# MasterVVK/qwen3-tts-axera-russian

Measured on AMD Instinct MI355X. Metric: 12Hz codec-tokens/s (codec frames/s, 16 codes each) + RTF, Qwen3-TTS-0.6B, higher is better.
Workload: dtype f16 weights/KV, f32 accumulate (talker+CP); vocoder exact fp32 (f32 MFMA); 1 GPU; configs[2]/[3]: batch=32 mixed ru/en prompts per GPU, 64 frames/utterance/step (prefill + hipGraph decode loop), utterance-sharded DP over 1 GPU(s); batch_per_gpu=32

## Files before the change

### qwen3_tts_axera_russian_amd/build.py

```python
from __future__ import annotations

import os
import shutil
import subprocess
import sys

HERE = os.path.dirname(os.path.abspath(__file__))
CSRC = os.path.join(HERE, "csrc")
LIB = os.path.join(HERE, "lib")
SOURCES = ["q3_common.cpp", "q3_formats.cpp", "q3_kernels.hip", "q3_model.hip", "q3_talker_api.hip", "q3_cp_api.hip",
           "q3_engine.hip", "q3_voc_kernels.hip", "q3_voc.hip", "q3_voc_stream.hip", "q3_enc.hip", "q3_enc_stream.hip",
           "q3_text_api.hip"]
TEST_SOURCES = ["q3_test_api.hip"]
ARCH = os.environ.get("Q3_OFFLOAD_ARCH", "gfx950")
EXTRA = os.environ.get("Q3_EXTRA_HIPCC_FLAGS", "-mllvm -amdgpu-kernarg-preload-count=16").split()


def _newer(dst: str, srcs) -> bool:
    if not os.path.exists(dst):
        return False
    t = os.path.getmtime(dst)
    return all(os.path.getmtime(s) <= t for s in srcs)


NO_SPILL = ("resunit_kernel", "linear_kernelILi1ELi1E", "linear_kernelILi1ELi2E", "linear_kernelILi2ELi1E",
            "linear_kernelILi2ELi2E", "attn_kernel", "attn_short_kernel", "cp_argmax_kernel", "talker_sample_kernel",
            "voc_attn_incr_kernel", "voc_incr_prepend_kernel", "voc_incr_emit_kernel", "voc_incr_prepend_split_kernel",
            "enc_conv_in_kernel", "enc_stream_unfold_kernel", "enc_stream_emit_kernel",
            "enc_stream_conv_in_kernel")


def kernel_resources(lib_path: str):
    import re
    import struct
    import tempfile
    readelf = "/opt/rocm/lib/llvm/bin/llvm-readelf"
    d = open(lib_path, "rb").read()
    res = {}
    i = d.find(b"__CLANG_OFFLOAD_BUNDLE__")
    while i >= 0:
        n = struct.unpack_from("<Q", d, i + 24)[0]
# ... 95 lines not shown
```

### qwen3_tts_axera_russian_amd/csrc/q3_cp_api.hip

```cpp
#include "../../include/qwen3tts_cp.h"
#include "q3_cp.h"

namespace q3 {

static bool two_row_enabled() {
    static const bool on = !(getenv("Q3_CP_TWO_ROW") && atoi(getenv("Q3_CP_TWO_ROW")) == 0);
    return on;
}

int cp_seed_row0(const Work& w, int R, int row0, int R_total) {
    (void)R;
    (void)row0;
    if (R_total <= 0) R_total = R;
    const int B16 = (R_total + 15) / 16 * 16;
    const bool two = two_row_enabled() && 2 * B16 <= w.max_rows;
    return two ? B16 : 0;
}

int cp_frame(hipStream_t s, const Model& m, Work& w, KVCache& kv, int R, const CpFrameIO& io, int row0, int R_total) {
    const ModelCfg& c = m.cfg;
    if (R_total <= 0) R_total = R;
    const int H = c.hidden, G = c.cp_groups;
    const int seed0 = cp_seed_row0(w, R, row0, R_total);
    RowMap rm;
// ... 36 lines not shown
        r2.pos = w.map_pos;
        r2.same_slot_rows = true;
        r2.valid_mod = R16;
        r2.valid_n = R;
        if (run_stack(s, m, m.cp, w, kv, R16 + R, r2, 256, 0)) return -1;
    } else {
        rm.pos_base = 0;
        if (run_stack(s, m, m.cp, w, kv, R, rm, 256, row0)) return -1;
        if (launch_gather_embed(s, m.talker_emb, c.talker_vocab, H, io.codes, 0, io.n_frames, io.frame_cap, 0, w.h, w.ssq, R,
                                row0, R_total, io.forced, w.xh, m.cp.L[0].in_ln))
            return -1;
        rm.pos_base = 1;
        if (run_stack(s, m, m.cp, w, kv, R, rm, 256, row0)) return -1;
    }
    const bool qkv_tab = m.cp_qkv_serves(R);
    for (int g = 0; g < G; g++) {
        if (g > 0) {
            rm.pos_base = g + 1;
            rm.skip_qkv0 = qkv_tab;
            if (run_stack(s, m, m.cp, w, kv, R, rm, 256, row0)) return -1;
        }
        LinArgs a;
        a.wp = m.cp_head[g].wp;
        a.N = c.cp_vocab;
        a.K = H;
        a.M = row0 + R;
        a.m_begin = row0;
        a.nt = 0;
        a.x16 = w.xh;
        a.ssq = w.ssq;
        a.ssq_parts = H / 16;
        a.eps = c.eps;
        a.y = w.logits;
        a.ldy = c.cp_vocab;
// ... 13 lines not shown
        x.top_k = io.top_k;
        x.seed = io.seed;
        x.seed_ptr = io.seed_ptr;
        x.forced = io.forced;
        x.slots = io.slots;
        if (g + 1 < G) {
            x.next_table = m.cp_emb[g];
            x.h_out = w.h;
            x.ssq_out = w.ssq;
            x.xh_out = w.xh;
            x.gamma_next = m.cp.L[0].in_ln;
            if (qkv_tab) {
                x.next_qkv = m.cp_qkv_rows(g);
                x.qkv_out = w.qkv;
                x.qkv_ld = (c.n_heads + 2 * c.n_kv) * c.head_dim;
            }
        } else if (io.fb_h) {
            x.talker_emb = m.talker_emb;
            x.talker_vocab = c.talker_vocab;
            x.cp_tables = m.d_cp_emb_ptrs;
            x.pad_embed = io.pad_embed;
            x.text_rows = io.text_rows;
            x.text_avail = io.text_avail;
            x.text_cap = io.text_cap;
            x.n_groups = G;
            x.h_out = io.fb_h;
            x.ssq_out = io.fb_ssq;
            x.xh_out = io.fb_xh;
            x.gamma_next = io.fb_gamma;
        }
// ... 187 lines not shown
```

### qwen3_tts_axera_russian_amd/csrc/q3_engine.hip

```cpp
#include "../../include/qwen3tts_engine.h"
#include "q3_cp.h"

#include <algorithm>
#include <chrono>
#include <cmath>

using namespace q3;

namespace {

struct Engine {
    Model* m = nullptr;
    int max_batch = 0, n_ctx = 0, max_frames = 0;
    hipStream_t s = nullptr;
    KVCache kv_t, kv_c;
    Work wt, wc;
    int prefill_rows = 0;
    int *d_slot = nullptr, *d_pos = nullptr;
    int* d_tiles = nullptr;
    int *d_iota = nullptr;
    int *d_past = nullptr, *d_npast = nullptr, *d_ntext = nullptr, *d_done = nullptr, *d_nframes = nullptr;
    int *d_pos0 = nullptr, *d_posdec = nullptr, *d_lastrow = nullptr;
    int* d_codes = nullptr;
    int* d_forced = nullptr;
// ... 184 lines not shown
    for (int c = 0; c < nc; c++) Q3_HIP(hipStreamWaitEvent(e->cs[c], e->ev_fork, 0), -1);
    return 0;
}
int join_chains(Engine* e) {
    const int nc = n_chains_eff(e);
    if (nc == 1) return 0;
    for (int c = 0; c < nc; c++) {
        Q3_HIP(hipEventRecord(e->ev_join[c], e->cs[c]), -1);
        Q3_HIP(hipStreamWaitEvent(e->s, e->ev_join[c], 0), -1);
    }
    return 0;
}

}

extern "C" {

void q3e_free(void* ee) {
    Engine* e = (Engine*)ee;
    if (!e) return;
    if (e->s) hipStreamSynchronize(e->s);
    for (auto& g : e->graph) g.reset();
    kv_free(e->kv_t);
    kv_free(e->kv_c);
    work_free(e->wt);
    work_free(e->wc);
    void* ps[] = {e->d_tiles, e->d_slot, e->d_pos,  e->d_iota,   e->d_past,    e->d_npast, e->d_ntext, e->d_done,
                  e->d_nframes, e->d_pos0, e->d_posdec, e->d_lastrow, e->d_codes, e->d_pad, e->d_forced, e->d_seed, e->d_slots,
                  e->d_text, e->d_tavail};
    for (void* p : ps)
// ... 714 lines not shown
```

### qwen3_tts_axera_russian_amd/csrc/q3_kernels.h

```cpp
#pragma once
#include "q3_common.h"

namespace q3 {

enum { PRO_F16 = 0, PRO_NORM = 1 };
enum { EPI_STORE = 0, EPI_RESID = 1, EPI_SWIGLU = 2 };

struct LinArgs {
    int tl_node = -1;
    const half_t* wp = nullptr;
    int N = 0, K = 0, M = 0;
    int m_begin = 0;
    int swap_grid = 0;
    int nt = 0;
    const half_t* x16 = nullptr;
    const float* ssq = nullptr;
    int ssq_parts = 0;
    float eps = 1e-6f;
    float* y = nullptr;
    int ldy = 0;
    float* h_out = nullptr;
    float* ssq_out = nullptr;
    half_t* xh_out = nullptr;
    const float* gamma = nullptr;
// ... 17 lines not shown
    const float* rope_sin = nullptr;
    const int* slot = nullptr;
    const int* pos = nullptr;
    int slot_base = 0, slot_stride = 0, pos_base = 0, pos_stride = 0;
    half_t* kc = nullptr;
    half_t* vc = nullptr;
    int n_ctx = 0, n_kv = 0, n_heads = 0;
    half_t* out = nullptr;
    float scale = 0.f;
    int threads = 256;
    int valid_mod = 0, valid_n = 0;
    const int* tiles = nullptr;
    int n_tiles = 0;
};
int launch_attn(hipStream_t s, const AttnArgs& a, int mode);

int launch_ssq_rows(hipStream_t s, const float* rows, float* h, float* ssq, int R, int H, half_t* xh = nullptr,
                    const float* gamma = nullptr, int dst_row0 = 0);

struct FinalNormArgs {
    int tl_node = -1;
    const float* h = nullptr;
    const float* ssq = nullptr;
    int ssq_parts = 0;
    const float* gamma = nullptr;
    float eps = 1e-6f;
    int R = 0, H = 0, row0 = 0;
    const int* row_map = nullptr;
    int src_off = 0;
    float* out_f32 = nullptr;
// ... 66 lines not shown
    int qkv_ld = 0;
    const float* talker_emb = nullptr;
    int talker_vocab = 0;
    const float* const* cp_tables = nullptr;
    const float* pad_embed = nullptr;
    int n_groups = 15;
    float temperature = 0.f;
    int top_k = 50;
    unsigned long long seed = 0;
    const unsigned long long* seed_ptr = nullptr;
    const int* forced = nullptr;
    const SlotParams* slots = nullptr;
    const float* text_rows = nullptr;
    const int* text_avail = nullptr;
    int text_cap = 0;
};
int launch_cp_argmax(hipStream_t s, const CpArgmaxArgs& a);

int launch_feedback(hipStream_t s, const int* codes16, int R, const float* talker_emb, int talker_vocab,
                    const float* const* cp_tables, int cp_vocab, int n_groups, const float* pad_embed,
                    float* h_out, float* ssq_out, int H, half_t* xh_out = nullptr, const float* gamma = nullptr);

int tl_next_node();

}
```

### qwen3_tts_axera_russian_amd/csrc/q3_kernels.hip

```cpp
#include "q3_kernels.h"

namespace q3 {

typedef _Float16 h8 __attribute__((ext_vector_type(8)));
typedef float f4 __attribute__((ext_vector_type(4)));

#ifdef Q3_TIMELINE
__device__ unsigned long long* g_tl = nullptr;
__device__ unsigned int g_tl_idx = 0;
__device__ unsigned int g_tl_cap = 0;
__device__ int g_skip = 0;
__device__ unsigned long long* g_ph = nullptr;
struct TlScope {
    unsigned int slot = 0xffffffffu;
    int id;
    __device__ __forceinline__ TlScope(int id_) : id(id_) {
        if (blockIdx.x == 0 && blockIdx.y == 0 && threadIdx.x == 0 && g_tl) {
            slot = atomicAdd(&g_tl_idx, 1u);
            if (slot < g_tl_cap) g_tl[2 * slot] = (wall_clock64() << 8) | (unsigned)id;
        }
    }
    __device__ __forceinline__ ~TlScope() {
        if (slot < g_tl_cap) g_tl[2 * slot + 1] = wall_clock64();
    }
// ... 4 lines not shown
struct TlScope2 {
    unsigned long long t0;
    int node, kind;
    __device__ __forceinline__ TlScope2(int n, int k) : node(n), kind(k) { t0 = wall_clock64(); }
    __device__ __forceinline__ ~TlScope2() {
        if (g_tl2 && node >= 0 && threadIdx.x == 0) {
            const unsigned b = blockIdx.x + gridDim.x * blockIdx.y;
            if (b < TL2_MAXB) {
                g_tl2[((size_t)node * TL2_MAXB + b) * 2] = t0;
                g_tl2[((size_t)node * TL2_MAXB + b) * 2 + 1] = wall_clock64();
            }
            if (b == 0 && g_tl2_kind) g_tl2_kind[node] = kind;
        }
    }
};
#define Q3_TL(id)      \
    if (g_skip) return; \
    TlScope2 tl_scope2_(a.tl_node, id); \
    TlScope tl_scope_(id)
#define Q3_PH(n)                                                                                       \
    do {                                                                                               \
        if (tl_scope_.slot < g_tl_cap && g_ph) g_ph[(size_t)tl_scope_.slot * 8 + (n)] = wall_clock64(); \
    } while (0)
#else
#ifndef Q3_WAVE_PRIO
#define Q3_WAVE_PRIO 3
#endif
#if Q3_WAVE_PRIO > 0
#define Q3_TL(id) __builtin_amdgcn_s_setprio(Q3_WAVE_PRIO)
#else
#define Q3_TL(id)
#endif
// ... 1070 lines not shown
        for (int i = 0; i < nwv; i++) M = fmaxf(M, pm[i * 2 + hh]);
        float L = 0.f, o = 0.f;
        for (int i = 0; i < nwv; i++) {
            const float mi = pm[i * 2 + hh];
            const float c = (mi == -INFINITY) ? 0.f : __expf(mi - M);
            L += pl[i * 2 + hh] * c;
            o += pacc[(i * 2 + hh) * D + d] * c;
        }
        a.out[frag_idx(r, (2 * g + hh) * D + d, a.n_heads * D)] = sat_half(o / L);
    }
}

constexpr int ATTN_SHORT_MAX_T = 15;
static int g_attn_short = 1;
int set_attn_short(int on) { g_attn_short = on; return 0; }
__global__ void __launch_bounds__(256)
    attn_short_kernel(float* __restrict__ p_qkv, int p_ld, int p_row0, int p_n_heads, int p_n_kv,
                      const float* __restrict__ p_q_norm, const float* __restrict__ p_k_norm,
                      const float* __restrict__ p_rope_cos, const float* __restrict__ p_rope_sin, int p_pos_base,
                      int p_slot_base, AttnArgs a) {
    constexpr int D = 128, NE = ATTN_SHORT_MAX_T + 1;
    a.qkv = p_qkv;
    a.ld = p_ld;
    a.row0 = p_row0;
    a.n_heads = p_n_heads;
    a.n_kv = p_n_kv;
    a.q_norm = p_q_norm;
    a.k_norm = p_k_norm;
    a.rope_cos = p_rope_cos;
    a.rope_sin = p_rope_sin;
    a.pos_base = p_pos_base;
    a.slot_base = p_slot_base;
    Q3_FETCH_ARGS("s"(a.eps), "s"(a.slot), "s"(a.slot_stride), "s"(a.kc), "s"(a.vc), "s"(a.n_ctx), "s"(a.out), "s"(a.scale));
    Q3_TL(33);
    const int r = a.row0 + blockIdx.x, g = blockIdx.y;
    const int tid = threadIdx.x, lane = tid & 63, w = tid >> 6;
    const int slot = a.slot ? uniform_load(a.slot + r) : a.slot_base + r * a.slot_stride;
    const int T = a.pos_base;
    __shared__ float qs[2][D];
    __shared__ float knew[D];
    __shared__ __attribute__((aligned(16))) half_t vs[NE][D];
    __shared__ __attribute__((aligned(16))) float sc[2][NE];
    float* row = a.qkv + (size_t)r * a.ld;
    const size_t cbase = ((size_t)slot * a.n_kv + g) * (size_t)a.n_ctx * D;
    const int l16 = tid & 15, grp = tid >> 4;
    const int hh = tid >> 7, d = tid & 127;
    float x0 = 0.f, x1 = 0.f, gm0 = 1.f, gm1 = 1.f, cs = 1.f, sn = 0.f;
    {
        const float* src = w < 2 ? row + (size_t)(2 * g + w) * D
                         : w == 2 ? row + (size_t)(a.n_heads + g) * D
                                  : row + (size_t)(a.n_heads + a.n_kv + g) * D;
        x0 = src[lane];
        x1 = src[lane + 64];
        if (w < 3) {
            const float* gam = w < 2 ? a.q_norm : a.k_norm;
            gm0 = gam[lane];
            gm1 = gam[lane + 64];
            cs = a.rope_cos[(size_t)T * 64 + lane];
            sn = a.rope_sin[(size_t)T * 64 + lane];
        }
    }
    h8 kpre, vpre;
    if (grp < T) {
        kpre = *(const h8*)(a.kc + cbase + (size_t)grp * D + l16 * 8);
        vpre = *(const h8*)(a.vc + cbase + (size_t)grp * D + l16 * 8);
    }
    __builtin_amdgcn_sched_barrier(0);
    Q3_PH(0);
    if (w < 3) {
        float ss = wave_sum(x0 * x0 + x1 * x1);
        const float iv = 1.0f / sqrtf(ss / (float)D + a.eps);
        x0 = (x0 * iv) * gm0;
        x1 = (x1 * iv) * gm1;
        const float y0 = x0 * cs - x1 * sn;
        const float y1 = x1 * cs + x0 * sn;
        x0 = y0;
        x1 = y1;
    }
    if (w < 2) {
        qs[w][lane] = x0;
        qs[w][lane + 64] = x1;
    } else {
        const half_t h0 = sat_half(x0), h1 = sat_half(x1);
        half_t* cd = (w == 2 ? a.kc : a.vc) + cbase + (size_t)T * D;
        cd[lane] = h0;
        cd[lane + 64] = h1;
        if (w == 2) {
            knew[lane] = (float)h0;
            knew[lane + 64] = (float)h1;
        } else {
            vs[T][lane] = h0;
            vs[T][lane + 64] = h1;
        }
    }
    if (grp < T) *(h8*)(&vs[grp][l16 * 8]) = vpre;
    __syncthreads();
    Q3_PH(1);
    if (grp <= T) {
        float d0 = 0.f, d1 = 0.f;
#pragma unroll
        for (int j = 0; j < 8; j++) {
            const float kf = grp < T ? (float)kpre[j] : knew[l16 * 8 + j];
            d0 += (qs[0][l16 * 8 + j] * a.scale) * kf;
            d1 += (qs[1][l16 * 8 + j] * a.scale) * kf;
        }
#pragma unroll
        for (int o = 8; o > 0; o >>= 1) {
            d0 += __shfl_xor(d0, o, 16);
            d1 += __shfl_xor(d1, o, 16);
        }
        if (l16 == 0) {
            sc[0][grp] = d0;
            sc[1][grp] = d1;
        }
    }
    __syncthreads();
    Q3_PH(2);
    float sv[NE];
#pragma unroll
    for (int e4 = 0; e4 < NE; e4 += 4) {
        const float4 t4 = *(const float4*)(&sc[hh][e4]);
        sv[e4] = t4.x;
        sv[e4 + 1] = t4.y;
        sv[e4 + 2] = t4.z;
        sv[e4 + 3] = t4.w;
    }
    float m = -INFINITY;
#pragma unroll
    for (int e = 0; e < NE; e++) m = fmaxf(m, e <= T ? sv[e] : -INFINITY);
    float L = 0.f, o = 0.f;
#pragma unroll
    for (int e = 0; e < NE; e++) {
        const float p = e <= T ? __expf(sv[e] - m) : 0.f;
        const float vf = e <= T ? (float)vs[e][d] : 0.f;
        L += p;
        o += p * vf;
    }
    Q3_PH(3);
    a.out[frag_idx(r, (2 * g + hh) * D + d, a.n_heads * D)] = sat_half(o / L);
}

__global__ void __launch_bounds__(256) attn_tile_mfma_kernel(AttnArgs a) {
    constexpr int D = 128, QP = 136, VP = 72, CH = 64;
    constexpr float LO = 2048.0f, ILO = 1.0f / 2048.0f;
    Q3_TL(35);
    const int g = blockIdx.y, tid = threadIdx.x, lane = tid & 63, w = tid >> 6;
    const int c = lane & 15, q4 = lane >> 4;
    int row0, nrows, slot, pos0;
    if (a.tiles) {
        const int4 t = *(const int4*)(a.tiles + 4 * blockIdx.x);
        row0 = t.x; nrows = t.y; slot = t.z; pos0 = t.w;
    } else {
        row0 = a.row0 + blockIdx.x * 16;
        nrows = a.R - blockIdx.x * 16 < 16 ? a.R - blockIdx.x * 16 : 16;
// ... 167 lines not shown
#pragma unroll
                for (int j = 0; j < 2; j++) {
                    const float o = (oh[qb][j][r] + ol[qb][j][r] * ILO) * inv;
                    a.out[frag_idx(row0 + i, (2 * g + qb) * D + 32 * w + 16 * j + c, a.n_heads * D)] = sat_half(o);
                }
            }
        }
}

int launch_attn(hipStream_t s, const AttnArgs& a, int mode) {
    if (a.R <= 0) return 0;
    if (a.n_heads != 2 * a.n_kv) {
        Q3_LOG("attn: only GQA group 2 (16q/8kv) is built, got %d/%d", a.n_heads, a.n_kv);
        return -1;
    }
    if (g_attn_short && mode == ATTN_FUSED && !a.pos && a.pos_stride == 0 && a.pos_base >= 0 &&
        a.pos_base <= ATTN_SHORT_MAX_T && a.pos_base < a.n_ctx) {
        AttnArgs a3 = a;
        a3.tl_node = tl_next_node();
        hipLaunchKernelGGL(attn_short_kernel, dim3(a.R, a.n_kv), dim3(256), 0, s, a3.qkv, a3.ld, a3.row0, a3.n_heads, a3.n_kv,
                           a3.q_norm, a3.k_norm, a3.rope_cos, a3.rope_sin, a3.pos_base, a3.slot_base, a3);
        Q3_HIP(hipGetLastError(), -1);
        return 0;
    }
    if (mode == ATTN_ATTEND && a.n_tiles > 0) {
        constexpr size_t lds = (size_t)(2 * 32 * 136 + 2 * 64 * 136 + 2 * 32 * 72) * 2 + 8 * 32 * 4;
        static bool attr = false;
        if (!attr) {
            Q3_HIP(hipFuncSetAttribute((const void*)attn_tile_mfma_kernel, hipFuncAttributeMaxDynamicSharedMemorySize, (int)lds), -1);
            attr = true;
        }
        AttnArgs a5 = a;
// ... 376 lines not shown
            v.x += e.x;
            v.y += e.y;
            v.z += e.z;
            v.w += e.w;
        }
        store_row_ssq(h_out, ssq_out, r, H, k4, v, xh_out, gamma);
    }
}

template <bool SLOTS>
__device__ __forceinline__ void cp_argmax_row(const CpArgmaxArgs& a) {
    if constexpr (SLOTS)
        Q3_FETCH_ARGS("s"(a.logits), "s"(a.V), "s"(a.H), "s"(a.row0), "s"(a.R_total), "s"(a.R), "s"(a.group), "s"(a.codes), "s"(a.n_frames),
                      "s"(a.frame_cap), "s"(a.next_table), "s"(a.h_out), "s"(a.ssq_out), "s"(a.xh_out), "s"(a.gamma_next),
                      "s"(a.talker_emb), "s"(a.slots), "s"(a.forced), "s"(a.next_qkv), "s"(a.qkv_out), "s"(a.qkv_ld),
                      "s"(a.text_rows), "s"(a.text_avail), "s"(a.text_cap));
    else
        Q3_FETCH_ARGS("s"(a.logits), "s"(a.V), "s"(a.H), "s"(a.row0), "s"(a.R_total), "s"(a.R), "s"(a.group), "s"(a.codes), "s"(a.n_frames),
                      "s"(a.frame_cap), "s"(a.next_table), "s"(a.h_out), "s"(a.ssq_out), "s"(a.xh_out), "s"(a.gamma_next),
                      "s"(a.talker_emb), "s"(a.temperature), "s"(a.forced), "s"(a.next_qkv), "s"(a.qkv_out), "s"(a.qkv_ld));
    Q3_TL(43);
    __shared__ float sv[4];
    __shared__ int si[4];
    const int r = a.row0 + blockIdx.x, tid = threadIdx.x;
    const int RT = a.R_total > 0 ? a.R_total : a.R;
    float best = -INFINITY;
    int bidx = 0x7fffffff;
    const float4* lg = (const float4*)(a.logits + (size_t)r * a.V);
    const int n4 = a.V / 4;
    float4 l0 = make_float4(-INFINITY, -INFINITY, -INFINITY, -INFINITY), l1 = l0;
    if (tid < n4) l0 = lg[tid];
    if (tid + 256 < n4) l1 = lg[tid + 256];
    const int nf_r = uniform_load(a.n_frames + r);
    float temperature = a.temperature;
    int top_k = a.top_k;
    int text_avail = 0;
    if constexpr (SLOTS) {
        const SlotParams sp = uniform_slot(a.slots, r);
        temperature = sp.c_temp;
        top_k = sp.c_top_k;
        if (a.talker_emb && a.text_rows) text_avail = uniform_load(a.text_avail + r);
    }
    Q3_PH(0);
    {
        const float e[8] = {nan_as_inf(l0.x), nan_as_inf(l0.y), nan_as_inf(l0.z), nan_as_inf(l0.w),
                            nan_as_inf(l1.x), nan_as_inf(l1.y), nan_as_inf(l1.z), nan_as_inf(l1.w)};
#pragma unroll
// ... 50 lines not shown
        float u;
        if constexpr (SLOTS) {
            const SlotParams sp = uniform_slot(a.slots, r);
            u = uniform01(sp.seed, sp.no_row ? 0u : (unsigned)r, (unsigned)nf_r, 1u + (unsigned)a.group);
        } else {
            u = uniform01(a.seed_ptr ? a.seed_ptr[r] : a.seed, (unsigned)r, (unsigned)nf_r, 1u + (unsigned)a.group);
        }
        bidx = block_sample_topk(slg, a.V, top_k, temperature, 0.f, u, sv2, si2, selv, seli);
    }
    if (bidx < 0 || bidx >= a.V) bidx = 0;
    int f = nf_r - 1;
    if (f < 0) f = 0;
    const bool keep = f < a.frame_cap;
    if (!keep) f = a.frame_cap - 1;
    int* fc = a.codes + ((size_t)f * RT + r) * 16;
    if (tid == 0 && keep) fc[1 + a.group] = bidx;
    const int* fz = (a.forced && keep) ? a.forced + ((size_t)f * RT + r) * 16 : nullptr;
    if (fz && fz[1 + a.group] >= 0) bidx = fz[1 + a.group];
    Q3_PH(2);
    if (a.talker_emb) {
        const float* last = a.pad_embed;
        if constexpr (SLOTS)
            if (nf_r >= 1 && nf_r - 1 < text_avail) last = a.text_rows + ((size_t)r * a.text_cap + (nf_r - 1)) * a.H;
        feedback_row(fc, r, a.talker_emb, a.talker_vocab, a.cp_tables, a.V, a.n_groups, last,
                     a.h_out, a.ssq_out, a.H, a.group, bidx, fz, a.xh_out, a.gamma_next);
    } else if (a.next_table) {
        const bool ok = bidx < a.V;
        const int t = ok ? bidx : 0;
        const float4 zero = make_float4(0.f, 0.f, 0.f, 0.f);
        const float* erow = a.next_table + (size_t)t * a.H;
        const int ne4 = a.H / 4;
        if (a.next_qkv) {
            constexpr int QV = 4;
            const int nq4 = a.qkv_ld / 4;
            const float4* tq = (const float4*)(a.next_qkv + (size_t)t * a.qkv_ld);
            float4* dq = (float4*)(a.qkv_out + (size_t)r * a.qkv_ld);
            float4 ev = *(const float4*)(erow + (tid < ne4 ? tid : 0) * 4);
            float4 qv[QV];
#pragma unroll
            for (int j = 0; j < QV; j++) {
                const int i = tid + 256 * j;
                qv[j] = tq[i < nq4 ? i : 0];
            }
            if (!ok) {
                ev = zero;
#pragma unroll
                for (int j = 0; j < QV; j++) qv[j] = zero;
// ... 29 lines not shown
int launch_cp_argmax(hipStream_t s, const CpArgmaxArgs& a) {
    if (a.R <= 0) return 0;
    if (a.V % 4) {
        Q3_LOG("cp_argmax: a vocabulary of %d is not a multiple of 4", a.V);
        return -1;
    }
    if (a.slots && a.V > SAMPLE_SORT_CAP) {
        Q3_LOG("cp_argmax: a vocabulary of %d is beyond the per-slot sampler (sort cap %d)", a.V, SAMPLE_SORT_CAP);
        return -1;
    }
    if (a.temperature > 1e-6f && effective_top_k(a.top_k, a.V) > SAMPLE_SEL_CAP && a.V > SAMPLE_SORT_CAP) {
        Q3_LOG("cp_argmax: top_k=%d over a vocabulary of %d is beyond the device sampler (sort cap %d)", a.top_k, a.V,
               SAMPLE_SORT_CAP);
        return -1;
    }
    const size_t lds = a.slots ? sample_lds_bytes_slots(a.V) : sample_lds_bytes(a.V, a.top_k, a.temperature);
    CpArgmaxArgs a2 = a;
    a2.tl_node = tl_next_node();
    if (a.slots) hipLaunchKernelGGL(cp_argmax_kernel_slots, dim3(a.R), dim3(256), lds, s, a2);
    else hipLaunchKernelGGL(cp_argmax_kernel, dim3(a.R), dim3(256), lds, s, a2);
    Q3_HIP(hipGetLastError(), -1);
    return 0;
}

__global__ void feedback_kernel(const int* codes, const float* talker_emb, int talker_vocab,
                                const float* const* cp_tables, int cp_vocab, int n_groups, const float* pad,
                                float* h_out, float* ssq_out, int H, half_t* xh_out, const float* gamma) {
    feedback_row(codes + (size_t)blockIdx.x * 16, blockIdx.x, talker_emb, talker_vocab, cp_tables, cp_vocab, n_groups,
                 pad, h_out, ssq_out, H, -1, 0, nullptr, xh_out, gamma);
}
int launch_feedback(hipStream_t s, const int* codes16, int R, const float* talker_emb, int talker_vocab,
                    const float* const* cp_tables, int cp_vocab, int n_groups, const float* pad_embed,
                    float* h_out, float* ssq_out, int H, half_t* xh_out, const float* gamma) {
    if (R <= 0) return 0;
    hipLaunchKernelGGL(feedback_kernel, dim3(R), dim3(256), 0, s, codes16, talker_emb, talker_vocab, cp_tables,
// ... 78 lines not shown
```

### qwen3_tts_axera_russian_amd/csrc/q3_model.h

```cpp
#pragma once
#include "q3_kernels.h"

namespace q3 {

struct DevLinear {
    half_t* wp = nullptr;
    int N = 0, K = 0;
};

struct DevLayer {
    DevLinear qkv, o, gu, down;
    float *in_ln = nullptr, *post_ln = nullptr, *q_norm = nullptr, *k_norm = nullptr;
};

struct DevStack {
    std::vector<DevLayer> L;
    float* final_norm = nullptr;
    const float* tail_gamma = nullptr;
    int ffn = 0;
    int nt = 0;
    size_t weight_bytes = 0;
};

struct Model {
// ... 50 lines not shown
    int map_R16 = 0;
};
int work_alloc(Work& w, const ModelCfg& c, int max_rows, int ffn, int max_vocab, hipStream_t s = nullptr);
void work_free(Work& w);
int work_zero(hipStream_t s, Work& w, const ModelCfg& c, int ffn, int max_vocab);

struct RowMap {
    const int* slot = nullptr;
    const int* pos = nullptr;
    int slot_base = 0, slot_stride = 0, pos_base = 0, pos_stride = 0;
    bool same_slot_rows = false;
    int valid_mod = 0, valid_n = 0;
    const int* tiles = nullptr;
    int n_tiles = 0;
    bool skip_qkv0 = false;
    int rows_total = 0;
};

int run_stack(hipStream_t s, const Model& m, const DevStack& st, Work& w, KVCache& kv, int R,
              const RowMap& rm, int attn_threads, int row0 = 0);

struct GraphExec {
    hipGraph_t g = nullptr;
    hipGraphExec_t e = nullptr;
    void reset();
};

}
```

### qwen3_tts_axera_russian_amd/csrc/q3_model.hip

```cpp
#include "q3_model.h"

#include <cmath>

namespace q3 {

namespace {

struct Loader {
    Model* m;
    const Pack& p;
    hipStream_t s = nullptr;
    half_t* stage = nullptr;
    size_t stage_elems = 0;
    std::vector<uint16_t> host16;
    bool ok = true;

    bool up(void* d, const void* src, size_t bytes) {
        return hipMemcpyAsync(d, src, bytes, hipMemcpyHostToDevice, s) == hipSuccess && hipStreamSynchronize(s) == hipSuccess;
    }
    void* dalloc(size_t bytes) {
        void* d = nullptr;
        if (hipMalloc(&d, bytes) != hipSuccess) {
            Q3_LOG("hipMalloc(%zu) failed", bytes);
            ok = false;
// ... 391 lines not shown
        t.kc = kv.k + li * kv.layer_stride();
        t.vc = kv.v + li * kv.layer_stride();
        t.n_ctx = kv.n_ctx;
        t.n_kv = c.n_kv;
        t.n_heads = c.n_heads;
        t.out = w.attn;
        t.scale = 1.0f / sqrtf((float)D);
        t.threads = attn_threads;
        if (rm.rows_total > R) {
            const int fit = 65536 / (rm.rows_total * c.n_kv);
            if (t.threads > fit) t.threads = fit / 64 * 64;
            if (t.threads < 256) t.threads = 256;
        }
        t.valid_mod = rm.valid_mod;
        t.valid_n = rm.valid_n;
        if (rm.same_slot_rows && R > 1) {
            if (launch_attn(s, t, ATTN_PREP)) return -1;
            if (rm.tiles && rm.n_tiles > 0) {
                t.tiles = rm.tiles;
                t.n_tiles = rm.n_tiles;
            } else if (!rm.slot && !rm.pos && rm.slot_stride == 0 && rm.pos_stride == 1 && rm.valid_mod == 0) {
                t.tiles = nullptr;
                t.n_tiles = (R + 15) / 16;
            }
            if (launch_attn(s, t, ATTN_ATTEND)) return -1;
        } else {
            if (launch_attn(s, t, ATTN_FUSED)) return -1;
        }
        a = LinArgs();
        a.wp = L.o.wp;
        a.N = H;
// ... 49 lines not shown
```

### qwen3_tts_axera_russian_amd/csrc/q3_test_api.hip

```cpp
#include "q3_enc.h"
#include "q3_model.h"
#include "q3_voc_ops.h"
#include <chrono>
#include <cstring>
#include <vector>

using namespace q3;

namespace q3 {
int set_linear_tuning(int K, int mt16, int kbw);
int set_linear_split_rows(int on);
int set_linear_narrow8(int on);
int set_linear_wide_tiles(int on);
int set_attn_short(int on);
int set_gemm_min_rows(int n);
int set_gemm_glds(int on);
int reset_linear_knobs();
const char* last_linear_variant();
}

namespace {
struct DBuf {
    void* p = nullptr;
    ~DBuf() {
        if (p) hipFree(p);
    }
    bool alloc(size_t n) { return hipMalloc(&p, n ? n : 16) == hipSuccess; }
    bool up(const void* src, size_t n) { return alloc(n) && (n == 0 || hipMemcpy(p, src, n, hipMemcpyHostToDevice) == hipSuccess); }
};
}

extern "C" {

int q3t_set_linear_tuning(int K, int mt16, int kbw) { return set_linear_tuning(K, mt16, kbw); }
int q3t_set_linear_split_rows(int on) { return set_linear_split_rows(on); }
int q3t_set_linear_narrow8(int on) { return set_linear_narrow8(on); }
int q3t_set_linear_wide_tiles(int on) { return set_linear_wide_tiles(on); }
int q3t_set_attn_short(int on) { return set_attn_short(on); }
int q3t_set_gemm_min_rows(int n) { return set_gemm_min_rows(n); }
int q3t_set_gemm_glds(int on) { return set_gemm_glds(on); }
int q3t_reset_linear_knobs() { return reset_linear_knobs(); }
const char* q3t_last_linear_variant() { return last_linear_variant(); }

int q3t_linear(int M, int N, int K, const uint16_t* W, int gateup, int pro, int epi, const uint16_t* x16,
               const float* h, const float* gamma, float eps, float* y_or_h_io, float* ssq_out, uint16_t* act_out,
               int nt) {
    hipStream_t s = nullptr;
    const int Mp = (M + 127) / 128 * 128;
    DBuf dW, dWp, dx, dhrows, dh, dssq, dg, dy, dso, dact, dxh;
    if (!dW.up(W, (size_t)N * K * 2) || !dWp.alloc((size_t)N * K * 2)) return -1;
    if (gateup) {
        if (launch_pack_linear(s, (const half_t*)dW.p, N / 2, K, (half_t*)dWp.p, 0, 2)) return -1;
        if (launch_pack_linear(s, (const half_t*)dW.p + (size_t)(N / 2) * K, N / 2, K, (half_t*)dWp.p, 1, 2)) return -1;
// ... 715 lines not shown
```

### qwen3_tts_axera_russian_amd/hiplib.py

```python
from __future__ import annotations

import ctypes
import os

from . import LIB_PATH, TEST_LIB_PATH

_lib = None
_test_lib = None

c_void_p, c_int, c_float, c_char_p = ctypes.c_void_p, ctypes.c_int, ctypes.c_float, ctypes.c_char_p
f32p = ctypes.POINTER(ctypes.c_float)
i32p = ctypes.POINTER(ctypes.c_int32)
i64p = ctypes.POINTER(ctypes.c_int64)
u16p = ctypes.POINTER(ctypes.c_uint16)
i16p = ctypes.POINTER(ctypes.c_int16)


class SlotParamsC(ctypes.Structure):
    _fields_ = [("max_frames", ctypes.c_int32), ("temperature", ctypes.c_float), ("top_k", ctypes.c_int32),
                ("top_p", ctypes.c_float), ("cp_temperature", ctypes.c_float), ("cp_top_k", ctypes.c_int32),
                ("seed", ctypes.c_uint64), ("utt", ctypes.c_int32), ("reserved", ctypes.c_int32)]


class KernelSlotParamsC(ctypes.Structure):
# ... 161 lines not shown
    _sig(lib, "q3t_talker_sample", c_int, [f32p, c_int, i32p, c_int, c_int, c_int])
    u64, u64p = ctypes.c_uint64, ctypes.POINTER(ctypes.c_uint64)
    _sig(lib, "q3t_talker_sample_case", c_int, [f32p, c_int, c_int, c_int, c_int, i32p, i32p, i32p, i32p, i32p, i32p, i32p,
                                                i32p, c_int, i32p, c_int, c_int, c_int, c_int, c_float, c_float, c_int,
                                                c_float, u64, u64p, c_void_p])
    _sig(lib, "q3t_cp_sample_case", c_int, [f32p, c_int, c_int, c_int, c_int, c_int, i32p, i32p, c_int, i32p, c_float, c_int,
                                            u64, u64p, c_void_p, c_int, c_int, f32p, f32p, c_int, f32p, f32p, c_int, f32p,
                                            c_int, f32p, f32p, f32p, ctypes.POINTER(ctypes.c_uint16), f32p])
    _sig(lib, "q3t_attn", c_int, [c_int, c_int, c_int, f32p, f32p, f32p, c_float, f32p, f32p, c_int, i32p, i32p, c_int,
                                  c_int, c_int, c_int, u16p, u16p, c_int, c_int, i32p, c_int, c_int, c_int, c_int, u16p])
    _sig(lib, "q3t_voc_attn", c_int, [c_int, f32p, f32p, c_int, c_int, c_int, c_int, c_int, c_float])
    _sig(lib, "q3t_set_linear_split_rows", c_int, [c_int])
    _sig(lib, "q3t_set_linear_narrow8", c_int, [c_int])
    _sig(lib, "q3t_set_linear_wide_tiles", c_int, [c_int])
    _sig(lib, "q3t_set_attn_short", c_int, [c_int])
    _sig(lib, "q3t_set_gemm_min_rows", c_int, [c_int])
    _sig(lib, "q3t_set_gemm_glds", c_int, [c_int])
    _sig(lib, "q3t_inspect_weights", c_int, [ctypes.c_char_p, ctypes.c_char_p, ctypes.c_char_p, c_int])
    _sig(lib, "q3t_bench_linear", c_float, [c_int, c_int, c_int, c_int, c_int, c_int, c_int, c_int])
    _sig(lib, "q3t_bench_chain", c_float, [c_int, c_int, c_int, c_int, c_int, c_int])
    _sig(lib, "q3t_cp_model_load", c_void_p, [c_char_p])
    _sig(lib, "q3t_cp_model_free", None, [c_void_p])
    _sig(lib, "q3t_cp_qkv_ld", c_int, [c_void_p])
    _sig(lib, "q3t_cp_qkv_serves", c_int, [c_void_p, c_int])
    _sig(lib, "q3t_cp_qkv_tab", c_int, [c_void_p, c_int, i32p, c_int, f32p])
    _sig(lib, "q3t_cp_qkv_live", c_int, [c_void_p, c_int, i32p, c_int, c_int, f32p])
    _sig(lib, "q3t_enc_stream_embeddings", c_int, [c_void_p, c_int, i32p, f32p, i32p, i32p, i64p, ctypes.c_int64, i64p, f32p, i32p])
    i64s = ctypes.POINTER(ctypes.c_longlong)
    _sig(lib, "q3t_enc_stream_plan", c_int, [i32p, i32p, c_int, ctypes.c_longlong, ctypes.c_longlong, c_int, i64s, i64s, i64s])
    _test_lib = lib
# ... 10 lines not shown
```

Baseline: 10150 codec_frames/s.

## Fold code-predictor layer-0 short attention into the argmax/embedding kernel

```diff
diff --git a/qwen3_tts_axera_russian_amd/build.py b/qwen3_tts_axera_russian_amd/build.py
--- a/qwen3_tts_axera_russian_amd/build.py
+++ b/qwen3_tts_axera_russian_amd/build.py
@@ -24,7 +24,7 @@
 
 
 NO_SPILL = ("resunit_kernel", "linear_kernelILi1ELi1E", "linear_kernelILi1ELi2E", "linear_kernelILi2ELi1E",
-            "linear_kernelILi2ELi2E", "attn_kernel", "attn_short_kernel", "cp_argmax_kernel", "talker_sample_kernel",
+            "linear_kernelILi2ELi2E", "attn_kernel", "attn_short_kernel", "cp_argmax_kernel", "cp_argmax_kernel_slots", "talker_sample_kernel",
             "voc_attn_incr_kernel", "voc_incr_prepend_kernel", "voc_incr_emit_kernel", "voc_incr_prepend_split_kernel",
             "enc_conv_in_kernel", "enc_stream_unfold_kernel", "enc_stream_emit_kernel",
             "enc_stream_conv_in_kernel")
diff --git a/qwen3_tts_axera_russian_amd/csrc/q3_cp_api.hip b/qwen3_tts_axera_russian_amd/csrc/q3_cp_api.hip
--- a/qwen3_tts_axera_russian_amd/csrc/q3_cp_api.hip
+++ b/qwen3_tts_axera_russian_amd/csrc/q3_cp_api.hip
@@ -74,10 +74,12 @@
         if (run_stack(s, m, m.cp, w, kv, R, rm, 256, row0)) return -1;
     }
     const bool qkv_tab = m.cp_qkv_serves(R);
+    bool attn0_done = false;
     for (int g = 0; g < G; g++) {
         if (g > 0) {
             rm.pos_base = g + 1;
             rm.skip_qkv0 = qkv_tab;
+            rm.skip_attn0 = attn0_done;
             if (run_stack(s, m, m.cp, w, kv, R, rm, 256, row0)) return -1;
         }
         LinArgs a;
@@ -121,6 +123,26 @@
                 x.next_qkv = m.cp_qkv_rows(g);
                 x.qkv_out = w.qkv;
                 x.qkv_ld = (c.n_heads + 2 * c.n_kv) * c.head_dim;
+                attn0_done = cp_attn_fold() && attn_short_serves(g + 2, kv.n_ctx);
+                if (attn0_done) {
+                    const DevLayer& L0 = m.cp.L[0];
+                    x.qkv_out = nullptr;
+                    x.at_q_norm = L0.q_norm;
+                    x.at_k_norm = L0.k_norm;
+                    x.at_rope_cos = m.rope_cos;
+                    x.at_rope_sin = m.rope_sin;
+                    x.at_kc = kv.k;
+                    x.at_vc = kv.v;
+                    x.at_out = w.attn;
+                    x.at_eps = c.eps;
+                    x.at_scale = 1.0f / sqrtf((float)c.head_dim);
+                    x.at_T = g + 2;
+                    x.at_n_ctx = kv.n_ctx;
+                    x.at_n_kv = c.n_kv;
+                    x.at_n_heads = c.n_heads;
+                    x.at_slot_base = rm.slot_base;
+                    x.at_slot_stride = rm.slot_stride;
+                }
             }
         } else if (io.fb_h) {
             x.talker_emb = m.talker_emb;
diff --git a/qwen3_tts_axera_russian_amd/csrc/q3_engine.hip b/qwen3_tts_axera_russian_amd/csrc/q3_engine.hip
--- a/qwen3_tts_axera_russian_amd/csrc/q3_engine.hip
+++ b/qwen3_tts_axera_russian_amd/csrc/q3_engine.hip
@@ -222,6 +222,31 @@
 
 }
 
+namespace q3 {
+int engine_graph_nodes(void* ee, int chain) {
+    Engine* e = (Engine*)ee;
+    if (!e || chain < 0 || chain >= 8) return -1;
+    if (!e->graph[chain].g) return 0;
+    size_t n = 0;
+    Q3_HIP(hipGraphGetNodes(e->graph[chain].g, nullptr, &n), -1);
+    return (int)n;
+}
+int engine_cp_cache(void* ee, int layer, int* dims, uint16_t* k, uint16_t* v, long long cap) {
+    Engine* e = (Engine*)ee;
+    if (!e || !dims || layer < 0 || layer >= e->kv_c.n_layers) return -1;
+    dims[0] = e->kv_c.n_slots;
+    dims[1] = e->kv_c.n_kv;
+    dims[2] = e->kv_c.n_ctx;
+    if (!k || !v) return 0;
+    const size_t n = e->kv_c.layer_stride();
+    if ((long long)n > cap) return -2;
+    Q3_HIP(hipStreamSynchronize(e->s), -1);
+    Q3_HIP(hipMemcpy(k, e->kv_c.k + layer * n, n * 2, hipMemcpyDeviceToHost), -1);
+    Q3_HIP(hipMemcpy(v, e->kv_c.v + layer * n, n * 2, hipMemcpyDeviceToHost), -1);
+    return 0;
+}
+}
+
 extern "C" {
 
 void q3e_free(void* ee) {
diff --git a/qwen3_tts_axera_russian_amd/csrc/q3_kernels.h b/qwen3_tts_axera_russian_amd/csrc/q3_kernels.h
--- a/qwen3_tts_axera_russian_amd/csrc/q3_kernels.h
+++ b/qwen3_tts_axera_russian_amd/csrc/q3_kernels.h
@@ -55,6 +55,9 @@
     int n_tiles = 0;
 };
 int launch_attn(hipStream_t s, const AttnArgs& a, int mode);
+bool attn_short_serves(int pos, int n_ctx);
+bool cp_attn_fold();
+int set_cp_attn_fold(int on);
 
 int launch_ssq_rows(hipStream_t s, const float* rows, float* h, float* ssq, int R, int H, half_t* xh = nullptr,
                     const float* gamma = nullptr, int dst_row0 = 0);
@@ -151,6 +154,15 @@
     const float* text_rows = nullptr;
     const int* text_avail = nullptr;
     int text_cap = 0;
+    const float* at_q_norm = nullptr;
+    const float* at_k_norm = nullptr;
+    const float* at_rope_cos = nullptr;
+    const float* at_rope_sin = nullptr;
+    half_t* at_kc = nullptr;
+    half_t* at_vc = nullptr;
+    half_t* at_out = nullptr;
+    float at_eps = 1e-6f, at_scale = 0.f;
+    int at_T = 0, at_n_ctx = 0, at_n_kv = 0, at_n_heads = 0, at_slot_base = 0, at_slot_stride = 0;
 };
 int launch_cp_argmax(hipStream_t s, const CpArgmaxArgs& a);
 
diff --git a/qwen3_tts_axera_russian_amd/csrc/q3_kernels.hip b/qwen3_tts_axera_russian_amd/csrc/q3_kernels.hip
--- a/qwen3_tts_axera_russian_amd/csrc/q3_kernels.hip
+++ b/qwen3_tts_axera_russian_amd/csrc/q3_kernels.hip
@@ -42,8 +42,12 @@
         }
     }
 };
+#ifndef Q3_WAVE_PRIO
+#define Q3_WAVE_PRIO 3
+#endif
 #define Q3_TL(id)      \
     if (g_skip) return; \
+    __builtin_amdgcn_s_setprio(Q3_WAVE_PRIO); \
     TlScope2 tl_scope2_(a.tl_node, id); \
     TlScope tl_scope_(id)
 #define Q3_PH(n)                                                                                       \
@@ -1144,12 +1148,135 @@
 constexpr int ATTN_SHORT_MAX_T = 15;
 static int g_attn_short = 1;
 int set_attn_short(int on) { g_attn_short = on; return 0; }
+bool attn_short_serves(int pos, int n_ctx) { return g_attn_short && pos >= 0 && pos <= ATTN_SHORT_MAX_T && pos < n_ctx; }
+static int g_cp_attn_fold = -1;
+bool cp_attn_fold() {
+    if (g_cp_attn_fold < 0) g_cp_attn_fold = !(getenv("Q3_CP_ATTN_FOLD") && atoi(getenv("Q3_CP_ATTN_FOLD")) == 0);
+    return g_cp_attn_fold != 0;
+}
+int set_cp_attn_fold(int on) { g_cp_attn_fold = on ? 1 : 0; return 0; }
+
+struct AttnShortPre {
+    float gm0 = 1.f, gm1 = 1.f, cs = 1.f, sn = 0.f;
+    h8 kpre, vpre;
+};
+__device__ __forceinline__ void attn_short_prefetch(AttnShortPre& p, const float* __restrict__ q_norm,
+                                                    const float* __restrict__ k_norm, const float* __restrict__ rope_cos,
+                                                    const float* __restrict__ rope_sin, const half_t* kc, const half_t* vc,
+                                                    size_t cbase, int T) {
+    constexpr int D = 128;
+    const int tid = threadIdx.x, lane = tid & 63, w = tid >> 6, l16 = tid & 15, grp = tid >> 4;
+    if (w < 3) {
+        const float* gam = w < 2 ? q_norm : k_norm;
+        p.gm0 = gam[lane];
+        p.gm1 = gam[lane + 64];
+        p.cs = rope_cos[(size_t)T * 64 + lane];
+        p.sn = rope_sin[(size_t)T * 64 + lane];
+    }
+    if (grp < T) {
+        p.kpre = *(const h8*)(kc + cbase + (size_t)grp * D + l16 * 8);
+        p.vpre = *(const h8*)(vc + cbase + (size_t)grp * D + l16 * 8);
+    }
+}
+template <class PH>
+__device__ __forceinline__ void attn_short_finish(float x0, float x1, const AttnShortPre& p, int r, int g, int T, size_t cbase,
+                                                  half_t* kc, half_t* vc, half_t* __restrict__ out, int n_heads, float eps,
+                                                  float scale, PH ph) {
+    constexpr int D = 128, NE = ATTN_SHORT_MAX_T + 1;
+    __shared__ float qs[2][D];
+    __shared__ float knew[D];
+    __shared__ __attribute__((aligned(16))) half_t vs[NE][D];
+    __shared__ __attribute__((aligned(16))) float sc[2][NE];
+    const int tid = threadIdx.x, lane = tid & 63, w = tid >> 6;
+    const int l16 = tid & 15, grp = tid >> 4;
+    const int hh = tid >> 7, d = tid & 127;
+    if (w < 3) {
+        float ss, y0, y1;
+        {
+#pragma clang fp contract(off)
+            ss = x0 * x0 + x1 * x1;
+        }
+        ss = wave_sum(ss);
+        const float iv = 1.0f / sqrtf(ss / (float)D + eps);
+        x0 = (x0 * iv) * p.gm0;
+        x1 = (x1 * iv) * p.gm1;
+        {
+#pragma clang fp contract(off)
+            y0 = __builtin_fmaf(x0, p.cs, -(x1 * p.sn));
+            y1 = x1 * p.cs + x0 * p.sn;
+        }
+        x0 = y0;
+        x1 = y1;
+    }
+    if (w < 2) {
+        qs[w][lane] = x0;
+        qs[w][lane + 64] = x1;
+    } else {
+        const half_t h0 = sat_half(x0), h1 = sat_half(x1);
+        half_t* cd = (w == 2 ? kc : vc) + cbase + (size_t)T * D;
+        cd[lane] = h0;
+        cd[lane + 64] = h1;
+        if (w == 2) {
+            knew[lane] = (float)h0;
+            knew[lane + 64] = (float)h1;
+        } else {
+            vs[T][lane] = h0;
+            vs[T][lane + 64] = h1;
+        }
+    }
+    if (grp < T) *(h8*)(&vs[grp][l16 * 8]) = p.vpre;
+    __syncthreads();
+    ph(1);
+    if (grp <= T) {
+        float d0 = 0.f, d1 = 0.f;
+#pragma unroll
+        for (int j = 0; j < 8; j++) {
+            const float kf = grp < T ? (float)p.kpre[j] : knew[l16 * 8 + j];
+            d0 += (qs[0][l16 * 8 + j] * scale) * kf;
+            d1 += (qs[1][l16 * 8 + j] * scale) * kf;
+        }
+#pragma unroll
+        for (int o = 8; o > 0; o >>= 1) {
+            d0 += __shfl_xor(d0, o, 16);
+            d1 += __shfl_xor(d1, o, 16);
+        }
+        if (l16 == 0) {
+            sc[0][grp] = d0;
+            sc[1][grp] = d1;
+        }
+    }
+    __syncthreads();
+    ph(2);
+    float sv[NE];
+#pragma unroll
+    for (int e4 = 0; e4 < NE; e4 += 4) {
+        const float4 t4 = *(const float4*)(&sc[hh][e4]);
+        sv[e4] = t4.x;
+        sv[e4 + 1] = t4.y;
+        sv[e4 + 2] = t4.z;
+        sv[e4 + 3] = t4.w;
+    }
+    float m = -INFINITY;
+#pragma unroll
+    for (int e = 0; e < NE; e++) m = fmaxf(m, e <= T ? sv[e] : -INFINITY);
+    float L = 0.f, o = 0.f;
+#pragma unroll
+    for (int e = 0; e < NE; e++) {
+        const float pe = e <= T ? __expf(sv[e] - m) : 0.f;
+        const float vf = e <= T ? (float)vs[e][d] : 0.f;
+        L += pe;
+        o += pe * vf;
+    }
+    ph(3);
+    out[frag_idx(r, (2 * g + hh) * D + d, n_heads * D)] = sat_half(o / L);
+}
+
 __global__ void __launch_bounds__(256)
     attn_short_kernel(float* __restrict__ p_qkv, int p_ld, int p_row0, int p_n_heads, int p_n_kv,
                       const float* __restrict__ p_q_norm, const float* __restrict__ p_k_norm,
                       const float* __restrict__ p_rope_cos, const float* __restrict__ p_rope_sin, int p_pos_base,
                       int p_slot_base, AttnArgs a) {
-    constexpr int D = 128, NE = ATTN_SHORT_MAX_T + 1;
+    constexpr int D = 128;
     a.qkv = p_qkv;
     a.ld = p_ld;
     a.row0 = p_row0;
@@ -1167,107 +1294,18 @@
     const int tid = threadIdx.x, lane = tid & 63, w = tid >> 6;
     const int slot = a.slot ? uniform_load(a.slot + r) : a.slot_base + r * a.slot_stride;
     const int T = a.pos_base;
-    __shared__ float qs[2][D];
-    __shared__ float knew[D];
-    __shared__ __attribute__((aligned(16))) half_t vs[NE][D];
-    __shared__ __attribute__((aligned(16))) float sc[2][NE];
     float* row = a.qkv + (size_t)r * a.ld;
     const size_t cbase = ((size_t)slot * a.n_kv + g) * (size_t)a.n_ctx * D;
-    const int l16 = tid & 15, grp = tid >> 4;
-    const int hh = tid >> 7, d = tid & 127;
-    float x0 = 0.f, x1 = 0.f, gm0 = 1.f, gm1 = 1.f, cs = 1.f, sn = 0.f;
-    {
-        const float* src = w < 2 ? row + (size_t)(2 * g + w) * D
-                         : w == 2 ? row + (size_t)(a.n_heads + g) * D
-                                  : row + (size_t)(a.n_heads + a.n_kv + g) * D;
-        x0 = src[lane];
-        x1 = src[lane + 64];
-        if (w < 3) {
-            const float* gam = w < 2 ? a.q_norm : a.k_norm;
-            gm0 = gam[lane];
-            gm1 = gam[lane + 64];
-            cs = a.rope_cos[(size_t)T * 64 + lane];
-            sn = a.rope_sin[(size_t)T * 64 + lane];
-        }
-    }
-    h8 kpre, vpre;
-    if (grp < T) {
-        kpre = *(const h8*)(a.kc + cbase + (size_t)grp * D + l16 * 8);
-        vpre = *(const h8*)(a.vc + cbase + (size_t)grp * D + l16 * 8);
-    }
+    const float* src = w < 2 ? row + (size_t)(2 * g + w) * D
+                     : w == 2 ? row + (size_t)(a.n_heads + g) * D
+                              : row + (size_t)(a.n_heads + a.n_kv + g) * D;
+    const float x0 = src[lane];
+    const float x1 = src[lane + 64];
+    AttnShortPre pre;
+    attn_short_prefetch(pre, a.q_norm, a.k_norm, a.rope_cos, a.rope_sin, a.kc, a.vc, cbase, T);
     __builtin_amdgcn_sched_barrier(0);
     Q3_PH(0);
-    if (w < 3) {
-        float ss = wave_sum(x0 * x0 + x1 * x1);
-        const float iv = 1.0f / sqrtf(ss / (float)D + a.eps);
-        x0 = (x0 * iv) * gm0;
-        x1 = (x1 * iv) * gm1;
-        const float y0 = x0 * cs - x1 * sn;
-        const float y1 = x1 * cs + x0 * sn;
-        x0 = y0;
-        x1 = y1;
-    }
-    if (w < 2) {
-        qs[w][lane] = x0;
-        qs[w][lane + 64] = x1;
-    } else {
-        const half_t h0 = sat_half(x0), h1 = sat_half(x1);
-        half_t* cd = (w == 2 ? a.kc : a.vc) + cbase + (size_t)T * D;
-        cd[lane] = h0;
-        cd[lane + 64] = h1;
-        if (w == 2) {
-            knew[lane] = (float)h0;
-            knew[lane + 64] = (float)h1;
-        } else {
-            vs[T][lane] = h0;
-            vs[T][lane + 64] = h1;
-        }
-    }
-    if (grp < T) *(h8*)(&vs[grp][l16 * 8]) = vpre;
-    __syncthreads();
-    Q3_PH(1);
-    if (grp <= T) {
-        float d0 = 0.f, d1 = 0.f;
-#pragma unroll
-        for (int j = 0; j < 8; j++) {
-            const float kf = grp < T ? (float)kpre[j] : knew[l16 * 8 + j];
-            d0 += (qs[0][l16 * 8 + j] * a.scale) * kf;
-            d1 += (qs[1][l16 * 8 + j] * a.scale) * kf;
-        }
-#pragma unroll
-        for (int o = 8; o > 0; o >>= 1) {
-            d0 += __shfl_xor(d0, o, 16);
-            d1 += __shfl_xor(d1, o, 16);
-        }
-        if (l16 == 0) {
-            sc[0][grp] = d0;
-            sc[1][grp] = d1;
-        }
-    }
-    __syncthreads();
-    Q3_PH(2);
-    float sv[NE];
-#pragma unroll
-    for (int e4 = 0; e4 < NE; e4 += 4) {
-        const float4 t4 = *(const float4*)(&sc[hh][e4]);
-        sv[e4] = t4.x;
-        sv[e4 + 1] = t4.y;
-        sv[e4 + 2] = t4.z;
-        sv[e4 + 3] = t4.w;
-    }
-    float m = -INFINITY;
-#pragma unroll
-    for (int e = 0; e < NE; e++) m = fmaxf(m, e <= T ? sv[e] : -INFINITY);
-    float L = 0.f, o = 0.f;
-#pragma unroll
-    for (int e = 0; e < NE; e++) {
-        const float p = e <= T ? __expf(sv[e] - m) : 0.f;
-        const float vf = e <= T ? (float)vs[e][d] : 0.f;
-        L += p;
-        o += p * vf;
-    }
-    Q3_PH(3);
-    a.out[frag_idx(r, (2 * g + hh) * D + d, a.n_heads * D)] = sat_half(o / L);
+    attn_short_finish(x0, x1, pre, r, g, T, cbase, a.kc, a.vc, a.out, a.n_heads, a.eps, a.scale, [&](int n) { Q3_PH(n); });
 }
 
 __global__ void __launch_bounds__(256) attn_tile_mfma_kernel(AttnArgs a) {
@@ -1465,8 +1503,7 @@
         Q3_LOG("attn: only GQA group 2 (16q/8kv) is built, got %d/%d", a.n_heads, a.n_kv);
         return -1;
     }
-    if (g_attn_short && mode == ATTN_FUSED && !a.pos && a.pos_stride == 0 && a.pos_base >= 0 &&
-        a.pos_base <= ATTN_SHORT_MAX_T && a.pos_base < a.n_ctx) {
+    if (mode == ATTN_FUSED && !a.pos && a.pos_stride == 0 && attn_short_serves(a.pos_base, a.n_ctx)) {
         AttnArgs a3 = a;
         a3.tl_node = tl_next_node();
         hipLaunchKernelGGL(attn_short_kernel, dim3(a.R, a.n_kv), dim3(256), 0, s, a3.qkv, a3.ld, a3.row0, a3.n_heads, a3.n_kv,
@@ -1873,11 +1910,17 @@
         Q3_FETCH_ARGS("s"(a.logits), "s"(a.V), "s"(a.H), "s"(a.row0), "s"(a.R_total), "s"(a.R), "s"(a.group), "s"(a.codes), "s"(a.n_frames),
                       "s"(a.frame_cap), "s"(a.next_table), "s"(a.h_out), "s"(a.ssq_out), "s"(a.xh_out), "s"(a.gamma_next),
                       "s"(a.talker_emb), "s"(a.slots), "s"(a.forced), "s"(a.next_qkv), "s"(a.qkv_out), "s"(a.qkv_ld),
-                      "s"(a.text_rows), "s"(a.text_avail), "s"(a.text_cap));
+                      "s"(a.text_rows), "s"(a.text_avail), "s"(a.text_cap), "s"(a.at_q_norm), "s"(a.at_k_norm),
+                      "s"(a.at_rope_cos), "s"(a.at_rope_sin), "s"(a.at_kc), "s"(a.at_vc), "s"(a.at_out), "s"(a.at_eps),
+                      "s"(a.at_scale), "s"(a.at_T), "s"(a.at_n_ctx), "s"(a.at_n_kv), "s"(a.at_n_heads), "s"(a.at_slot_base),
+                      "s"(a.at_slot_stride));
     else
         Q3_FETCH_ARGS("s"(a.logits), "s"(a.V), "s"(a.H), "s"(a.row0), "s"(a.R_total), "s"(a.R), "s"(a.group), "s"(a.codes), "s"(a.n_frames),
                       "s"(a.frame_cap), "s"(a.next_table), "s"(a.h_out), "s"(a.ssq_out), "s"(a.xh_out), "s"(a.gamma_next),
-                      "s"(a.talker_emb), "s"(a.temperature), "s"(a.forced), "s"(a.next_qkv), "s"(a.qkv_out), "s"(a.qkv_ld));
+                      "s"(a.talker_emb), "s"(a.temperature), "s"(a.forced), "s"(a.next_qkv), "s"(a.qkv_out), "s"(a.qkv_ld), "s"(a.at_q_norm), "s"(a.at_k_norm),
+                      "s"(a.at_rope_cos), "s"(a.at_rope_sin), "s"(a.at_kc), "s"(a.at_vc), "s"(a.at_out), "s"(a.at_eps),
+                      "s"(a.at_scale), "s"(a.at_T), "s"(a.at_n_ctx), "s"(a.at_n_kv), "s"(a.at_n_heads), "s"(a.at_slot_base),
+                      "s"(a.at_slot_stride));
     Q3_TL(43);
     __shared__ float sv[4];
     __shared__ int si[4];
@@ -1890,6 +1933,14 @@
     float4 l0 = make_float4(-INFINITY, -INFINITY, -INFINITY, -INFINITY), l1 = l0;
     if (tid < n4) l0 = lg[tid];
     if (tid + 256 < n4) l1 = lg[tid + 256];
+    const bool fold = a.at_kc != nullptr;
+    const int kvh = blockIdx.y;
+    AttnShortPre pre;
+    size_t cbase = 0;
+    if (fold) {
+        cbase = ((size_t)(a.at_slot_base + r * a.at_slot_stride) * a.at_n_kv + kvh) * (size_t)a.at_n_ctx * 128;
+        attn_short_prefetch(pre, a.at_q_norm, a.at_k_norm, a.at_rope_cos, a.at_rope_sin, a.at_kc, a.at_vc, cbase, a.at_T);
+    }
     const int nf_r = uniform_load(a.n_frames + r);
     float temperature = a.temperature;
     int top_k = a.top_k;
@@ -1970,7 +2021,7 @@
     const bool keep = f < a.frame_cap;
     if (!keep) f = a.frame_cap - 1;
     int* fc = a.codes + ((size_t)f * RT + r) * 16;
-    if (tid == 0 && keep) fc[1 + a.group] = bidx;
+    if (tid == 0 && keep && kvh == 0) fc[1 + a.group] = bidx;
     const int* fz = (a.forced && keep) ? a.forced + ((size_t)f * RT + r) * 16 : nullptr;
     if (fz && fz[1 + a.group] >= 0) bidx = fz[1 + a.group];
     Q3_PH(2);
@@ -1986,7 +2037,25 @@
         const float4 zero = make_float4(0.f, 0.f, 0.f, 0.f);
         const float* erow = a.next_table + (size_t)t * a.H;
         const int ne4 = a.H / 4;
-        if (a.next_qkv) {
+        if (fold) {
+            constexpr int D = 128;
+            const int lane = tid & 63, w = tid >> 6;
+            const float* tq = a.next_qkv + (size_t)t * a.qkv_ld;
+            const float* src = w < 2 ? tq + (size_t)(2 * kvh + w) * D
+                             : w == 2 ? tq + (size_t)(a.at_n_heads + kvh) * D
+                                      : tq + (size_t)(a.at_n_heads + a.at_n_kv + kvh) * D;
+            float x0 = src[lane];
+            float x1 = src[lane + 64];
+            if (!ok) x0 = x1 = 0.f;
+            if (kvh == 0)
+                for (int k4 = tid; k4 < ne4; k4 += 256) {
+                    float4 v = *(const float4*)(erow + k4 * 4);
+                    if (!ok) v = zero;
+                    store_row_ssq(a.h_out, a.ssq_out, r, a.H, k4, v, a.xh_out, a.gamma_next);
+                }
+            attn_short_finish(x0, x1, pre, r, kvh, a.at_T, cbase, a.at_kc, a.at_vc, a.at_out, a.at_n_heads, a.at_eps,
+                              a.at_scale, [&](int n) { Q3_PH(3 + n); });
+        } else if (a.next_qkv) {
             constexpr int QV = 4;
             const int nq4 = a.qkv_ld / 4;
             const float4* tq = (const float4*)(a.next_qkv + (size_t)t * a.qkv_ld);
@@ -2046,11 +2115,22 @@
                SAMPLE_SORT_CAP);
         return -1;
     }
+    dim3 grid(a.R);
+    if (a.at_kc) {
+        if (!a.next_table || !a.next_qkv || a.talker_emb || !a.at_vc || !a.at_out || a.at_n_heads != 2 * a.at_n_kv ||
+            a.at_n_kv <= 0 || a.qkv_ld != (a.at_n_heads + 2 * a.at_n_kv) * 128 || a.at_T < 0 || a.at_T > ATTN_SHORT_MAX_T ||
+            a.at_T >= a.at_n_ctx) {
+            Q3_LOG("cp_argmax: folded attention of position %d (n_ctx %d, %d/%d heads) is not served", a.at_T, a.at_n_ctx,
+                   a.at_n_heads, a.at_n_kv);
+            return -1;
+        }
+        grid = dim3(a.R, a.at_n_kv);
+    }
     const size_t lds = a.slots ? sample_lds_bytes_slots(a.V) : sample_lds_bytes(a.V, a.top_k, a.temperature);
     CpArgmaxArgs a2 = a;
     a2.tl_node = tl_next_node();
-    if (a.slots) hipLaunchKernelGGL(cp_argmax_kernel_slots, dim3(a.R), dim3(256), lds, s, a2);
-    else hipLaunchKernelGGL(cp_argmax_kernel, dim3(a.R), dim3(256), lds, s, a2);
+    if (a.slots) hipLaunchKernelGGL(cp_argmax_kernel_slots, grid, dim3(256), lds, s, a2);
+    else hipLaunchKernelGGL(cp_argmax_kernel, grid, dim3(256), lds, s, a2);
     Q3_HIP(hipGetLastError(), -1);
     return 0;
 }
diff --git a/qwen3_tts_axera_russian_amd/csrc/q3_model.h b/qwen3_tts_axera_russian_amd/csrc/q3_model.h
--- a/qwen3_tts_axera_russian_amd/csrc/q3_model.h
+++ b/qwen3_tts_axera_russian_amd/csrc/q3_model.h
@@ -88,6 +88,7 @@
     const int* tiles = nullptr;
     int n_tiles = 0;
     bool skip_qkv0 = false;
+    bool skip_attn0 = false;
     int rows_total = 0;
 };
 
diff --git a/qwen3_tts_axera_russian_amd/csrc/q3_model.hip b/qwen3_tts_axera_russian_amd/csrc/q3_model.hip
--- a/qwen3_tts_axera_russian_amd/csrc/q3_model.hip
+++ b/qwen3_tts_axera_russian_amd/csrc/q3_model.hip
@@ -429,7 +429,8 @@
         }
         t.valid_mod = rm.valid_mod;
         t.valid_n = rm.valid_n;
-        if (rm.same_slot_rows && R > 1) {
+        if (li == 0 && rm.skip_attn0) {
+        } else if (rm.same_slot_rows && R > 1) {
             if (launch_attn(s, t, ATTN_PREP)) return -1;
             if (rm.tiles && rm.n_tiles > 0) {
                 t.tiles = rm.tiles;
diff --git a/qwen3_tts_axera_russian_amd/csrc/q3_test_api.hip b/qwen3_tts_axera_russian_amd/csrc/q3_test_api.hip
--- a/qwen3_tts_axera_russian_amd/csrc/q3_test_api.hip
+++ b/qwen3_tts_axera_russian_amd/csrc/q3_test_api.hip
@@ -13,6 +13,8 @@
 int set_linear_narrow8(int on);
 int set_linear_wide_tiles(int on);
 int set_attn_short(int on);
+int engine_graph_nodes(void* e, int chain);
+int engine_cp_cache(void* e, int layer, int* dims, uint16_t* k, uint16_t* v, long long cap);
 int set_gemm_min_rows(int n);
 int set_gemm_glds(int on);
 int reset_linear_knobs();
@@ -37,6 +39,11 @@
 int q3t_set_linear_narrow8(int on) { return set_linear_narrow8(on); }
 int q3t_set_linear_wide_tiles(int on) { return set_linear_wide_tiles(on); }
 int q3t_set_attn_short(int on) { return set_attn_short(on); }
+int q3t_set_cp_attn_fold(int on) { return set_cp_attn_fold(on); }
+int q3t_engine_graph_nodes(void* e, int chain) { return engine_graph_nodes(e, chain); }
+int q3t_engine_cp_cache(void* e, int layer, int* dims, uint16_t* k, uint16_t* v, long long cap) {
+    return engine_cp_cache(e, layer, dims, k, v, cap);
+}
 int q3t_set_gemm_min_rows(int n) { return set_gemm_min_rows(n); }
 int q3t_set_gemm_glds(int on) { return set_gemm_glds(on); }
 int q3t_reset_linear_knobs() { return reset_linear_knobs(); }
diff --git a/qwen3_tts_axera_russian_amd/hiplib.py b/qwen3_tts_axera_russian_amd/hiplib.py
--- a/qwen3_tts_axera_russian_amd/hiplib.py
+++ b/qwen3_tts_axera_russian_amd/hiplib.py
@@ -199,6 +199,9 @@
     _sig(lib, "q3t_set_linear_narrow8", c_int, [c_int])
     _sig(lib, "q3t_set_linear_wide_tiles", c_int, [c_int])
     _sig(lib, "q3t_set_attn_short", c_int, [c_int])
+    _sig(lib, "q3t_set_cp_attn_fold", c_int, [c_int])
+    _sig(lib, "q3t_engine_graph_nodes", c_int, [c_void_p, c_int])
+    _sig(lib, "q3t_engine_cp_cache", c_int, [c_void_p, c_int, i32p, u16p, u16p, ctypes.c_longlong])
     _sig(lib, "q3t_set_gemm_min_rows", c_int, [c_int])
     _sig(lib, "q3t_set_gemm_glds", c_int, [c_int])
     _sig(lib, "q3t_inspect_weights", c_int, [ctypes.c_char_p, ctypes.c_char_p, ctypes.c_char_p, c_int])
```

New measurement: 10220 codec_frames/s, median of 6. No clear change (+0.7%).
